# Shuijing725/CrowdNav_Prediction_AttnGraph

Hardware: AMD Instinct MI355X
Metric: env-steps/sec (sim+policy fwd) at 20 humans (higher is better)
Workload: dtype f32 (big GEMMs as bf16x3 split-precision MFMA, fp32 accumulate); 1 GPU; BASELINE configs[1]: CrowdSimVarNum-v0, 20 humans, 4096 parallel envs per GPU, HH+HR attention on, policy forward + ORCA sim step + auto-reset per step; envs_per_gpu=4096, humans=20, parallelism=dp1 (envs sharded, no rollout collective), policy_init=orthogonal, torch.manual_seed(425), sampled_actions=True, side_stream_tail=inline, dephase_steps=240

## Files before the change

crowdnav_prediction_attngraph_amd/csrc/common.h:

```cpp
#pragma once
#include <hip/hip_runtime.h>

#include <cstdarg>
#include <cstdint>
#include <cstdio>

#include "crowdnav_hip.h"

void cn_set_error(const char *fmt, ...);

#define CN_HIP(expr)                                                                                         \
    do {                                                                                                     \
        hipError_t cn_e_ = (expr);                                                                           \
        if (cn_e_ != hipSuccess) {                                                                           \
            cn_set_error("%s failed: %s (%s:%d)", #expr, hipGetErrorString(cn_e_), __FILE__, __LINE__);      \
            return CN_ERR_HIP;                                                                               \
        }                                                                                                    \
    } while (0)

#define CN_CHECK_LAUNCH() CN_HIP(hipGetLastError())

#define CN_REQUIRE(cond, ...)               \
    do {                                    \
        if (!(cond)) {                      \
// ... 82 lines not shown
    v = fmaxf(v, wv_dpp<0x118, 0xf>(v, I));
    v = fmaxf(v, wv_dpp<0x142, 0xa>(v, I));
    v = fmaxf(v, wv_dpp<0x143, 0xc>(v, I));
    return wv_readlane(v, 63);
}
__device__ __forceinline__ float wv_sum(float v)
{
    v += wv_dpp<0x111, 0xf>(v, 0.0f);
    v += wv_dpp<0x112, 0xf>(v, 0.0f);
    v += wv_dpp<0x114, 0xf>(v, 0.0f);
    v += wv_dpp<0x118, 0xf>(v, 0.0f);
    v += wv_dpp<0x142, 0xa>(v, 0.0f);
    v += wv_dpp<0x143, 0xc>(v, 0.0f);
    return wv_readlane(v, 63);
}
__device__ __forceinline__ double wv_min(double v)
{
#pragma unroll
    for (int o = 32; o > 0; o >>= 1) v = fmin(v, __shfl_xor(v, o, 64));
    return v;
}
__device__ __forceinline__ double wv_sum(double v)
{
#pragma unroll
    for (int o = 32; o > 0; o >>= 1) v += __shfl_xor(v, o, 64);
    return v;
}
```

crowdnav_prediction_attngraph_amd/csrc/det_math.h:

```cpp
#pragma once
#include "common.h"

#include <cmath>

namespace {

__device__ __forceinline__ double poly_sin(double x)
{
    const double S1 = -1.66666666666666324348e-01, S2 = 8.33333333332248946124e-03, S3 = -1.98412698298579493134e-04,
                 S4 = 2.75573137070700676789e-06, S5 = -2.50507602534068634195e-08, S6 = 1.58969099521155010221e-10;
    const double z = x * x, w = z * z;
    const double r = S2 + z * (S3 + z * S4) + z * w * (S5 + z * S6);
    const double v = z * x;
    return x + v * (S1 + z * r);
}
__device__ __forceinline__ double poly_cos(double x)
{
    const double C1 = 4.16666666666666019037e-02, C2 = -1.38888888888741095749e-03, C3 = 2.48015872894767294178e-05,
                 C4 = -2.75573143513906633035e-07, C5 = 2.08757232129817482790e-09, C6 = -1.13596475577881948265e-11;
    const double z = x * x;
    double w = z * z;
    const double r = z * (C1 + z * (C2 + z * C3)) + (w * w) * (C4 + z * (C5 + z * C6));
    const double hz = 0.5 * z;
    w = 1.0 - hz;
// ... 54 lines not shown
    }
    const double s = f / (2.0 + f);
    const double z = s * s;
    const double w = z * z;
    const double t1 = w * (Lg2 + w * (Lg4 + w * Lg6));
    const double t2 = z * (Lg1 + w * (Lg3 + w * (Lg5 + w * Lg7)));
    const double R = t2 + t1;
    const int i = (hx - 0x6147a) | (0x6b851 - hx);
    if (i > 0) {
        const double hfsq = 0.5 * f * f;
        return k == 0 ? f - (hfsq - s * (hfsq + R)) : dk * ln2_hi - ((hfsq - (s * (hfsq + R) + dk * ln2_lo)) - f);
    }
    return k == 0 ? f - s * (f - R) : dk * ln2_hi - ((s * (f - R) - dk * ln2_lo) - f);
}

__device__ __forceinline__ bool in_fov(const cn_env_config &c, double fov, double px1, double py1, double vx1, double vy1, double theta1,
                                       double px2, double py2)
{
    double fx, fy;
    if (c.kinematics == CN_KIN_UNICYCLE) det_sincos(theta1, fy, fx);
    else if (vx1 == 0.0 && vy1 == 0.0) { fx = __double_as_longlong(vx1) < 0 ? -1.0 : 1.0; fy = 0.0; }
    else { const double nv = sqrt(vx1 * vx1 + vy1 * vy1); fx = vx1 / nv; fy = vy1 / nv; }
    const double dx = px2 - px1, dy = py2 - py1;
    const double n12 = sqrt(dx * dx + dy * dy);
    double d = fx * (dx / n12) + fy * (dy / n12);
    d = d < -1.0 ? -1.0 : (d > 1.0 ? 1.0 : d);
    const double half = M_PI * fov / 2.0;
    double thr = -1.0;
    if (half < M_PI) { double sn; det_sincos(half, sn, thr); }
    return d >= thr;
}
// ... 3 lines not shown
```

crowdnav_prediction_attngraph_amd/csrc/env_dev.h:

```cpp
#pragma once
#include "common.h"

namespace {

constexpr int MT_N = 624;
constexpr float RVO_EPS = 0.00001f;

struct Lp3Hdr { int32_t agent, nn, line_fail; float rx, ry, radius; };

struct EnvDev {
    cn_env_config cfg;
    int E, H, D, P;
    int I, R;
    int64_t seed_base;
    double *hum;
    double *rob;
    double *lhs;
    double *ftraj;
    int32_t *step_counter;
    uint64_t *case_counter;
    double *ep_ret;
    int32_t *ep_cnt;
    double *shared_nd;
    uint8_t *sim_valid;
// ... 26 lines not shown
    int32_t *obs_max;
    uint8_t *sim_n;
    uint8_t *rob_sim_n;
    int32_t *pred_id;
    int32_t *max_pid;
    uint8_t *last_obs;
    int32_t *lp3_cnt;
    struct Lp3Hdr *lp3_hdr;
    float4 *lp3_lines;
    double *desired_v;
    double *wheel;
    unsigned long long *stamp;
};
static EnvDev stamped(const EnvDev &d, int kernel_id) { EnvDev c = d; c.stamp = cn_stamp_slot(kernel_id); return c; }

__device__ __forceinline__ int crowd_size(const EnvDev &s, int e) { return s.nh ? s.nh[e] : s.H; }

constexpr int CN_MAX_PLACEMENT_ATTEMPTS = 1 << 16;

enum { F_PX = 0, F_PY, F_VX, F_VY, F_GX, F_GY, F_RAD, F_VPREF };
enum { R_PX = 0, R_PY, R_VX, R_VY, R_GX, R_GY, R_THETA, R_POT };

}
```

crowdnav_prediction_attngraph_amd/csrc/env_sim.hip:

```cpp
#include "common.h"
#include "env_dev.h"
#include "det_math.h"
#include "orca.h"
#include "mt19937.h"
#include "episode.h"

#include <cmath>
#include <cstdio>
#include <cstdlib>
#include <cstring>
#include <new>

namespace {

__global__ __launch_bounds__(64) void env_reset_kernel(EnvDev s, cn_obs ob, int with_obs)
{
    const int lane = threadIdx.x;
    const int e = blockIdx.x;
    Rng R{MT_N, false};
    Robot rb{};
    Lane h{};
    h.rad = s.cfg.human_radius;
    double shared_nd = s.cfg.orca_neighbor_dist;
    int n = s.H;
    if (e == 0 && lane == 0) *s.lp3_cnt = 0;
    const bool nx_ready = s.nx_ready[e] != 0;
// ... 62 lines not shown
    Rng R{MT_N, false};
    Robot rb;
    Lane h;
    load_env(s, e, lane, rb, h);
    double shared_nd = s.shared_nd[e];
    const bool was_reset = s.pend[e] != 0;
    const int n = crowd_size(s, e);
    write_obs(s, e, lane, n, was_reset, rb, h, ob, was_reset ? 0 : s.step_counter[e]);
    if (!was_reset) post_obs_updates(s, R, e, lane, n, s.step_counter[e], rb, h, shared_nd);
    if (lane == 0) s.pend[e] = 0;
    store_env(s, e, lane, rb, h);
    if (lane == 0) s.shared_nd[e] = shared_nd;
    rng_store(R, s, e, lane);
}

template <bool SPLIT, int W = 1, bool DEFER = false>
__global__ __launch_bounds__(64 * W, W > 1 ? 2 : 4) void env_step_kernel(EnvDev s, const float *actions, cn_obs ob, float *reward_out,
                                                      uint8_t *done_out, uint8_t *info_out, double *ep_ret_out, int32_t *ep_len_out, float *not_done_out)
{
    const CnStampScope stamp_scope(s.stamp);
    const int lane = threadIdx.x & 63;
    const int e = blockIdx.x;
    if constexpr (W > 1) {
        if (threadIdx.x >= 64) { coop_helper_loop<W>(lane, __builtin_amdgcn_readfirstlane((int)(threadIdx.x >> 6))); return; }
    }
    const cn_env_config &c = s.cfg;
    const int H = s.H;
    const int lj = lane < H ? lane : 0;
    int n = crowd_size(s, e);
    Rng R{MT_N, false};
    Robot rb;
    Lane h;
    load_env(s, e, lane, rb, h);
    double shared_nd = s.shared_nd[e];
    int step_counter = s.step_counter[e];
    float ax = actions[2 * e], ay = actions[2 * e + 1];
    const float hax = s.hact[(size_t)e * 2 * H + lj], hay = s.hact[(size_t)e * 2 * H + H + lj];
    double ep_ret_in = s.ep_ret[e];
    int ep_cnt_in = s.ep_cnt[e];
    int nx_ready_in = s.nx_ready[e];
    uint64_t case_counter = s.case_counter[e];
// ... 107 lines not shown
            const bool hidden = c.human_fov < 2.0 ? !in_fov(c, c.human_fov, h.px, h.py, h.vx, h.vy, 0.0, ox, oy) : (ox == h.px && oy == h.py);
            if (hidden) { ox = 7.0; oy = 7.0; if (j < n) orad = c.human_radius; }
            const double dx = h.px - ox, dy = h.py - oy;
            const double d = sqrt(dx * dx + dy * dy);
            const double f = c.sf_A * det_exp((h.rad + orad - d) / c.sf_B);
            if (j != lane) { ivx += f * (dx / d); ivy += f * (dy / d); }
        }
        const double nvx = h.vx + (curr_dvx + ivx) * c.time_step, nvy = h.vy + (curr_dvy + ivy) * c.time_step;
        const double act_norm = sqrt(nvx * nvx + nvy * nvy);
        if (act_norm > h.vpref) { sfx = nvx / act_norm * h.vpref; sfy = nvy / act_norm * h.vpref; }
        else { sfx = nvx; sfy = nvy; }
    }
    const double cdx = h.px - rb.px, cdy = h.py - rb.py;
    const double closest = isH ? sqrt(cdx * cdx + cdy * cdy) - h.rad - c.robot_radius : INFINITY;
    const bool collision = wv_any(closest < 0.0);
    const double dmin = wv_min(closest);
    const double goal_dist = norm2(rb.px - rb.gx, rb.py - rb.gy);
    const bool reaching_goal = goal_dist < (c.kinematics == CN_KIN_UNICYCLE ? 0.6 : c.robot_radius);
    const double global_time = (double)step_counter * c.time_step;
    double reward;
    int done, info;
    const bool test_phase = c.phase == CN_PHASE_TEST;
    bool danger_cond = dmin < c.discomfort_dist;
    double min_danger = 0.0, rf_truth = 0.0;
    if (test_phase) {
        const double *tre = s.tr + (size_t)e * (s.R + 1) * 4 * H;
        const bool seen = isH && held(seen_before) != 0;
        double best = INFINITY;
        for (int k = 1; k <= s.P; ++k) {
            if (isH) {
                const double fx = (seen ? tre[(k * s.I * 4 + 0) * H + lane] : 15.0) - rb.px, fy = (seen ? tre[(k * s.I * 4 + 1) * H + lane] : 15.0) - rb.py;
// ... 249 lines not shown
}

static int truth_rollout_and_obs(cn_env_batch *env, const cn_obs *obs, hipStream_t st)
{
    if (int rc = truth_rollout(env, st)) return rc;
    hipLaunchKernelGGL(env_obs_kernel, dim3(env->d.E), dim3(64), 0, st, env->d, *obs);
    CN_CHECK_LAUNCH();
    return CN_OK;
}

static bool lane_path_of(const cn_env_batch *env)
{
    const int slots = env->d.H + (env->d.cfg.robot_visible ? 1 : 0);
    return env->d.cfg.humans_policy == CN_HUMANS_ORCA && slots <= 32 && env->d.cfg.human_fov >= 2.0;
}

static bool dense_crowd(cn_env_batch *env)
{
    const cn_env_config &cf = env->d.cfg;
    const double zone = 2.0 * (2.0 * (cf.randomize_attributes ? 0.5 : cf.human_radius) + cf.discomfort_dist) * env->d.H;
    static const int coop_env = getenv("CN_ENV_COOP") ? atoi(getenv("CN_ENV_COOP")) : -1;
    static const int coop_after = getenv("CN_COOP_AFTER") ? atoi(getenv("CN_COOP_AFTER")) : COOP_AFTER;
    env->d.coop_after = coop_after;
    return coop_env >= 0 ? coop_env != 0 : zone > 0.9 * 2.0 * M_PI * cf.circle_radius;
}

static int launch_post(cn_env_batch *env, hipStream_t on)
{
    hipLaunchKernelGGL(env_post_kernel<4>, dim3(env->d.E), dim3(256), 0, on, stamped(env->d, CN_K_OTHER));
    CN_CHECK_LAUNCH();
// ... 302 lines not shown
    if (!env->orca_ready && !env->tail_pending) { if (int rc = prefetch_orca(env, st, nullptr)) return rc; }
    if (int rc = sync_side(env, st)) return rc;
    if (env->d.cfg.predict_truth) {
        hipLaunchKernelGGL(env_step_kernel<true>, dim3(env->d.E), dim3(64), 0, st, stamped(env->d, CN_K_ENV_STEP), actions, *obs, reward, done, info, ep_return, ep_len, not_done);
        CN_CHECK_LAUNCH();
        if (int rc = truth_rollout_and_obs(env, obs, st)) return rc;
    } else {
        const bool coop = dense_crowd(env);
        const bool defer = coop && !lane_path_of(env) && env->d.cfg.humans_policy == CN_HUMANS_ORCA;
        if (defer) {
            CN_HIP(hipMemsetAsync(env->d.post_cnt, 0, 4, st));
            hipLaunchKernelGGL((env_step_kernel<false, 1, true>), dim3(env->d.E), dim3(64), 0, st, stamped(env->d, CN_K_ENV_STEP), actions, *obs, reward, done, info, ep_return, ep_len, not_done);
            env->post_deferred = true;
        }
        else if (coop) hipLaunchKernelGGL((env_step_kernel<false, 4>), dim3(env->d.E), dim3(256), 0, st, stamped(env->d, CN_K_ENV_STEP), actions, *obs, reward, done, info, ep_return, ep_len, not_done);
        else hipLaunchKernelGGL(env_step_kernel<false>, dim3(env->d.E), dim3(64), 0, st, stamped(env->d, CN_K_ENV_STEP), actions, *obs, reward, done, info, ep_return, ep_len, not_done);
        CN_CHECK_LAUNCH();
    }
    return prefetch_orca(env, st, obs);
}

extern "C" int cn_env_join(cn_env_batch *env, void *stream)
{
    CN_REQUIRE(env, "cn_env_join: null handle");
    return sync_side(env, (hipStream_t)stream);
}

extern "C" int cn_env_get_state(cn_env_batch *env, double *humans, double *robot, void *stream)
{
    CN_REQUIRE(env, "cn_env_get_state: null handle");
// ... 138 lines not shown
```

crowdnav_prediction_attngraph_amd/csrc/episode.h:

```cpp
#pragma once
#include "env_dev.h"
#include "det_math.h"
#include "mt19937.h"

namespace {

struct Lane {
    double px, py, vx, vy, gx, gy, rad, vpref;
    double l0, l1, l2, l3, l4;
    uint8_t simv;
};
struct Robot { double px, py, vx, vy, gx, gy, theta, pot; };

__device__ __forceinline__ double norm2(double x, double y) { return sqrt(x * x + y * y); }
__device__ __forceinline__ bool closer_than(double x, double y, double d)
{
    const double q = x * x + y * y, dd = d * d;
    if (q < dd * (1.0 - 0x1p-48)) return true;
    if (q > dd * (1.0 + 0x1p-48)) return false;
    return sqrt(q) < d;
}

__device__ __forceinline__ double wv_readlane_d(double v, int lane_uniform)
{
    const long long b = __double_as_longlong(v);
    const unsigned lo = (unsigned)__builtin_amdgcn_readlane((int)(unsigned)(b & 0xffffffffll), lane_uniform);
    const unsigned hi = (unsigned)__builtin_amdgcn_readlane((int)(unsigned)((unsigned long long)b >> 32), lane_uniform);
    return __longlong_as_double((long long)(((unsigned long long)hi << 32) | lo));
}

constexpr int coop_c(int W) { return W <= 4 ? 4 : (W <= 8 ? 2 : 1); }
template <int W>
struct CoopLds {
    static constexpr int NE = W - 1;
    static constexpr int C = coop_c(W);
    static constexpr int NG = NE * C;
    static constexpr int NB1 = (384 * NG + 623) / MT_N;
    static constexpr int BW = MT_N * (NB1 + 1) + 227;
    int cmd;
    int verdict;
    int kind, n_pairs, max_att;
    int pos0, attempt0;
    float circle_radius, vp;
// ... 71 lines not shown
        const float2 lo = Q.plo[k];
#pragma unroll
        for (int cc = 0; cc < C; ++cc) {
            const f2 ax = xx[cc] - f2{pq.x, pq.y}, ay = yy[cc] - f2{pq.z, pq.w};
            const f2 d = (ax * ax + ay * ay) - f2{lo.x, lo.y};
            m[cc] = fminf(m[cc], fminf(d.x, d.y));
        }
    }
#pragma unroll
    for (int cc = 0; cc < C; ++cc) {
        const uint64_t take = __ballot(!(m[cc] < 0.0f) || att0 + 64 * (p * C + cc) + lane >= max_att);
        if (lane == 0) Q.take[round & 1][p * C + cc] = take;
    }
}

template <int W = 1>
__device__ __forceinline__ void place_by_rejection(const EnvDev &s, Rng &R, int lane, int kind, double radius, double vp, double md_r, int n_list, int skip,
                                                   const Robot &rb, const Lane &h, double &out_x, double &out_y)
{
    const cn_env_config &c = s.cfg;
    const int max_att = c.max_placement_attempts > 0 ? c.max_placement_attempts : CN_MAX_PLACEMENT_ATTEMPTS;
    auto make = [&](double u0, double u1, double u2, double &x, double &y) {
        const double angle = u0 * M_PI * 2.0;
        const double nx = kind == 0 ? (0.0 + (1.0 - 0.0) * u1) * 2.0 : (u1 - 0.5) * vp;
        const double ny = kind == 0 ? (0.0 + (1.0 - 0.0) * u2) * 2.0 : (u2 - 0.5) * vp;
        double sn, cs;
        det_sincos(angle, sn, cs);
        x = c.circle_radius * cs + nx;
        y = c.circle_radius * sn + ny;
    };
    const double md_l = radius + h.rad + c.discomfort_dist, dd_l = md_l * md_l;
    const double lo_l = dd_l * (1.0 - 0x1p-48), hi_l = dd_l * (1.0 + 0x1p-48);
    const double ddr = md_r * md_r, lo_r = ddr * (1.0 - 0x1p-48), hi_r = ddr * (1.0 + 0x1p-48);
    auto collides_exact = [&](double x, double y) {
        bool coll = norm2(x - rb.px, y - rb.py) < md_r || norm2(x - rb.gx, y - rb.gy) < md_r;
// ... 290 lines not shown
#endif
            __syncthreads();
            unsigned long long any = 0ull;
            for (int p = 0; p < NG; ++p) any |= Q.take[round & 1][p];
            if (any) {
                __syncthreads();
                if (Q.verdict) break;
            }
            bprev = (g0 + 384 * NG - 1) / MT_N;
            g0 += 384 * NG;
            attempt += 64 * NG;
        }
    }
}

template <int W = 1>
__device__ __forceinline__ void gen_human(const EnvDev &s, Rng &R, int lane, int slot, int n_existing, const Robot &rb, Lane &h, double &shared_nd)
{
    const cn_env_config &c = s.cfg;
    double radius = c.human_radius, vpref = c.human_v_pref;
    if (c.randomize_attributes) {
        shared_nd = rng_uniform(R, lane, 5.0, 10.0);
        vpref = rng_uniform(R, lane, 0.5, 1.5);
        radius = rng_uniform(R, lane, 0.3, 0.5);
    }
    double px, py;
    const double md_r = c.kinematics == CN_KIN_UNICYCLE ? c.circle_radius / 2.0 : radius + c.robot_radius + c.discomfort_dist;
    place_by_rejection<W>(s, R, lane, 0, radius, 0.0, md_r, n_existing, -1, rb, h, px, py);
    if (lane == slot) {
        h.px = px; h.py = py; h.gx = -px; h.gy = -py; h.vx = 0.0; h.vy = 0.0; h.rad = radius; h.vpref = vpref;
        h.simv = 0;
    }
}

template <int W = 1>
__device__ __forceinline__ void change_goals(const EnvDev &s, Rng &R, int lane, int n, const Robot &rb, Lane &h, int only = -1)
{
    const cn_env_config &c = s.cfg;
    const int H = n;
    for (int i = only >= 0 ? only : 0; i < (only >= 0 ? only + 1 : H); ++i) {
        double vp_i = __shfl(h.vpref, i, 64);
        const double rad_i = __shfl(h.rad, i, 64);
        if (only < 0 && vp_i == 0.0) continue;
        if (vp_i == 0.0) vp_i = 1.0;
        if (rng_double(R, lane) <= (only >= 0 ? c.end_goal_change_chance : c.goal_change_chance)) {
            double gx, gy;
            place_by_rejection<W>(s, R, lane, 1, rad_i, vp_i, rad_i + c.robot_radius + c.discomfort_dist, H, i, rb, h, gx, gy);
            if (lane == i) { h.gx = gx; h.gy = gy; }
        }
    }
}

__device__ __forceinline__ bool robot_sees(const cn_env_config &c, const Robot &rb, bool present, double hpx, double hpy, double hrad)
{
    const double dx = rb.px - hpx, dy = rb.py - hpy;
    bool vis = present && !(dx == 0.0 && dy == 0.0) && (norm2(dx, dy) - c.robot_radius - hrad <= c.sensor_range);
    if (c.robot_fov < 2.0) vis = vis && in_fov(c, c.robot_fov, rb.px, rb.py, rb.vx, rb.vy, rb.theta, hpx, hpy);
    return vis;
}

__device__ __forceinline__ void write_obs(const EnvDev &s, int e, int lane, int n, bool reset, const Robot &rb, Lane &h, const cn_obs &ob, int step_counter)
{
    const cn_env_config &c = s.cfg;
    const int H = s.H, D = s.D, P = s.P;
    const bool isH = lane < n, isRow = lane < H;
    const bool vis = robot_sees(c, rb, isH, h.px, h.py, h.rad);
    const uint64_t vmask = __ballot(vis);
    const int num_visible = __popcll(vmask);
    if (s.vis && isRow) s.vis[(size_t)e * H + lane] = vis ? 1 : 0;
    if (s.nh && c.env_kind != CN_ENV_PRED && lane == 0) {
        s.obs_cnt[e] = num_visible;
        s.obs_max[e] = vmask ? 63 - __clzll((long long)vmask) : -1;
    }
    const double prev_vx = h.l2, prev_vy = h.l3;
    if (vis) { h.l0 = h.px; h.l1 = h.py; h.l2 = h.vx; h.l3 = h.vy; h.l4 = h.rad; }
    else if (isH && reset) { h.l0 = 15.0; h.l1 = 15.0; h.l2 = 0.0; h.l3 = 0.0; h.l4 = 0.3; }
    else if (isH) { h.l0 = h.l0 + h.l2 * c.time_step; h.l1 = h.l1 + h.l3 * c.time_step; }
    if (lane == 0) {
// ... 18 lines not shown
            se[1] = (float)pid;
            se[2] = vis ? (float)h.l0 : INFINITY;
            se[3] = vis ? (float)h.l1 : INFINITY;
            if (ob.visible_masks) ob.visible_masks[(size_t)e * H + lane] = vis ? 1 : 0;
        }
        if (lane == 0 && omask) s.max_pid[e] = base + __popcll(omask);
        return;
    }
    const double ex = h.l0 - rb.px, ey = h.l1 - rb.py;
    const bool do_sort = c.sort_humans && c.env_kind != CN_ENV_PRED_GST;
    int row = lane;
    if (do_sort) {
        const double key = vis ? sqrt(ex * ex + ey * ey) : INFINITY;
        int rank = 0;
        for (int m = 0; m < H; ++m) {
            const double km = __shfl(key, m, 64);
            rank += (km < key || (km == key && m < lane)) ? 1 : 0;
        }
        row = rank;
    }
    if (isRow) {
        float *se = ob.spatial_edges + ((size_t)e * H + row) * D;
        if (c.env_kind == CN_ENV_VARNUM) {
            se[0] = vis ? (float)ex : 15.0f;
            se[1] = vis ? (float)ey : 15.0f;
        } else {
            double *ft = s.ftraj ? s.ftraj + (size_t)e * P * 2 * H : nullptr;
            const double *tre = c.predict_truth ? s.tr + (size_t)e * (s.R + 1) * 4 * H : nullptr;
            for (int k = 0; k <= P; ++k) {
                double fx = 15.0, fy = 15.0;
                if (vis && tre && k >= 1) {
// ... 10 lines not shown
                    se[2 * k + 1] = vis ? (float)(fy - rb.py) : 15.0f;
                } else {
                    se[2 * k] = vis ? (float)ex : 15.0f;
                    se[2 * k + 1] = vis ? (float)ey : 15.0f;
                }
            }
        }
        if (ob.visible_masks) {
            uint8_t *vm = ob.visible_masks + (size_t)e * H;
            if (do_sort) vm[lane] = lane < num_visible ? 1 : 0;
            else vm[lane] = vis ? 1 : 0;
        }
    }
}

__device__ __forceinline__ void gen_episode_head(const EnvDev &s, Rng &R, int e, int lane, uint64_t case_counter, Robot &rb, int &n)
{
    const cn_env_config &c = s.cfg;
    const uint64_t offset = c.phase == CN_PHASE_TRAIN ? 2000ull : (c.phase == CN_PHASE_VAL ? 0ull : 1000ull);
    const uint64_t seed = offset + case_counter + (uint64_t)(s.seed_base + e);
    rng_seed(R, (uint32_t)seed, lane);
    double px, py, gx, gy;
    if (c.kinematics == CN_KIN_UNICYCLE) {
        const double angle = rng_uniform(R, lane, 0.0, M_PI * 2.0);
        double sn, cs;
        det_sincos(angle, sn, cs);
        px = c.arena_size * cs; py = c.arena_size * sn;
        for (;;) {
            gx = rng_uniform(R, lane, -c.arena_size, c.arena_size);
            gy = rng_uniform(R, lane, -c.arena_size, c.arena_size);
            if (norm2(px - gx, py - gy) >= 4.0) break;
        }
        rb.theta = rng_uniform(R, lane, 0.0, 2.0 * M_PI);
        n = rng_randint(R, lane, 1, c.human_num + c.human_num_range + 1);
    } else {
        for (;;) {
            px = rng_uniform(R, lane, -c.arena_size, c.arena_size);
            py = rng_uniform(R, lane, -c.arena_size, c.arena_size);
            gx = rng_uniform(R, lane, -c.arena_size, c.arena_size);
            gy = rng_uniform(R, lane, -c.arena_size, c.arena_size);
            if (norm2(px - gx, py - gy) >= 8.0) break;
        }
        rb.theta = M_PI / 2.0;
        n = rng_randint(R, lane, c.human_num - c.human_num_range, c.human_num + c.human_num_range + 1);
    }
    rb.px = px; rb.py = py; rb.gx = gx; rb.gy = gy; rb.vx = 0.0; rb.vy = 0.0;
}
__device__ __forceinline__ void gen_episode(const EnvDev &s, Rng &R, int e, int lane, uint64_t case_counter, Robot &rb, Lane &h, double &shared_nd, int &n)
{
    gen_episode_head(s, R, e, lane, case_counter, rb, n);
    for (int i = 0; i < n; ++i) gen_human(s, R, lane, i, i, rb, h, shared_nd);
    rb.pot = -fabs(norm2(rb.gx - rb.px, rb.gy - rb.py));
}

__device__ __forceinline__ void finish_reset(const EnvDev &s, int e, int lane, int n, uint64_t case_counter, Robot &rb, Lane &h, const cn_obs &ob, bool with_obs = true)
{
    const cn_env_config &c = s.cfg;
    h.l0 = h.l1 = h.l2 = h.l3 = h.l4 = 0.0;
    const uint64_t case_size = c.phase == CN_PHASE_TRAIN ? (4294967295ull - 2000ull) : (c.phase == CN_PHASE_VAL ? c.val_size : c.test_size);
    if (lane == 0) {
        s.case_counter[e] = (case_counter + (uint64_t)c.nenv) % case_size;
        s.step_counter[e] = 0; s.ep_ret[e] = 0.0; s.ep_cnt[e] = 0;
        if (s.nh) { s.obs_cnt[e] = 0; s.obs_max[e] = -1; }
        if (s.max_pid) s.max_pid[e] = n;
        if (s.wheel) { s.wheel[(size_t)e * 4 + 2] = 0.0; s.wheel[(size_t)e * 4 + 3] = 0.0; }
    }
    if (s.pred_id && lane < s.H) { s.pred_id[(size_t)e * s.H + lane] = lane; s.last_obs[(size_t)e * s.H + lane] = 0; }
    if (with_obs) write_obs(s, e, lane, n, true, rb, h, ob, 0);
}

__device__ __forceinline__ void do_reset(const EnvDev &s, Rng &R, int e, int lane, bool nx_ready, uint64_t case_counter, Robot &rb, Lane &h,
                                         double &shared_nd, int &n, const cn_obs &ob, bool with_obs = true)
{
    if (nx_ready) {
        rng_sync();
        mt_dma(R.mt, s.nx_mt + (size_t)e * MT_N, lane);
        const int pos = s.nx_mt_pos[e];
        n = s.nx_nh ? s.nx_nh[e] : s.H;
        const int H = s.H;
        const int lj = lane < H ? lane : 0;
        const double *hum = s.nx_hum + (size_t)e * 8 * H;
        h.px = hum[F_PX * H + lj]; h.py = hum[F_PY * H + lj]; h.vx = 0.0; h.vy = 0.0;
        h.gx = hum[F_GX * H + lj]; h.gy = hum[F_GY * H + lj]; h.rad = hum[F_RAD * H + lj]; h.vpref = hum[F_VPREF * H + lj];
        h.simv = 0;
        const double *r = s.nx_rob + (size_t)e * 8;
        rb.px = r[R_PX]; rb.py = r[R_PY]; rb.vx = 0.0; rb.vy = 0.0; rb.gx = r[R_GX]; rb.gy = r[R_GY]; rb.theta = r[R_THETA]; rb.pot = r[R_POT];
        shared_nd = s.nx_shared_nd[e];
        mt_dma_wait();
        R.pos = pos;
        R.loaded = true;
        rng_sync();
        if (lane == 0) s.nx_ready[e] = 0;
    } else {
        gen_episode(s, R, e, lane, case_counter, rb, h, shared_nd, n);
    }
    finish_reset(s, e, lane, n, case_counter, rb, h, ob, with_obs);
}

__device__ __forceinline__ void load_env(const EnvDev &s, int e, int lane, Robot &rb, Lane &h)
{
    const int H = s.H;
    const int lj = lane < H ? lane : 0;
    const double *hum = s.hum + (size_t)e * 8 * H;
    h.px = hum[F_PX * H + lj]; h.py = hum[F_PY * H + lj]; h.vx = hum[F_VX * H + lj]; h.vy = hum[F_VY * H + lj];
    h.gx = hum[F_GX * H + lj]; h.gy = hum[F_GY * H + lj]; h.rad = hum[F_RAD * H + lj]; h.vpref = hum[F_VPREF * H + lj];
    const double *l = s.lhs + (size_t)e * 5 * H;
    h.l0 = l[lj]; h.l1 = l[H + lj]; h.l2 = l[2 * H + lj]; h.l3 = l[3 * H + lj]; h.l4 = l[4 * H + lj];
    h.simv = s.sim_valid[(size_t)e * H + lj];
    const double *r = s.rob + (size_t)e * 8;
    rb.px = r[R_PX]; rb.py = r[R_PY]; rb.vx = r[R_VX]; rb.vy = r[R_VY]; rb.gx = r[R_GX]; rb.gy = r[R_GY]; rb.theta = r[R_THETA]; rb.pot = r[R_POT];
}
__device__ __forceinline__ void store_env(const EnvDev &s, int e, int lane, const Robot &rb, const Lane &h)
{
    const int H = s.H;
    if (lane < H) {
        double *hum = s.hum + (size_t)e * 8 * H;
        hum[F_PX * H + lane] = h.px; hum[F_PY * H + lane] = h.py; hum[F_VX * H + lane] = h.vx; hum[F_VY * H + lane] = h.vy;
        hum[F_GX * H + lane] = h.gx; hum[F_GY * H + lane] = h.gy; hum[F_RAD * H + lane] = h.rad; hum[F_VPREF * H + lane] = h.vpref;
        double *l = s.lhs + (size_t)e * 5 * H;
        l[lane] = h.l0; l[H + lane] = h.l1; l[2 * H + lane] = h.l2; l[3 * H + lane] = h.l3; l[4 * H + lane] = h.l4;
        s.sim_valid[(size_t)e * H + lane] = h.simv;
    }
    if (lane == 0) {
        double *r = s.rob + (size_t)e * 8;
        r[R_PX] = rb.px; r[R_PY] = rb.py; r[R_VX] = rb.vx; r[R_VY] = rb.vy; r[R_GX] = rb.gx; r[R_GY] = rb.gy; r[R_THETA] = rb.theta; r[R_POT] = rb.pot;
    }
}

template <int W = 1>
__device__ __forceinline__ void pregen_env(const EnvDev &s, int e, int lane, long long budget, Rng &R)
{
    if (s.nx_ready[e]) return;
    const long long t0 = wall_clock64();
    const int H = s.H;
    int prog = s.nx_prog[e];
    if (prog > 0 && s.nx_case[e] != s.case_counter[e]) prog = 0;
    Robot rb{};
    Lane h{};
    h.rad = s.cfg.human_radius;
    double shared_nd = s.shared_nd[e];
    int n = H;
    if (prog == 0) {
        const uint64_t case_counter = s.case_counter[e];
        gen_episode_head(s, R, e, lane, case_counter, rb, n);
        if (lane == 0) s.nx_case[e] = case_counter;
// ... 26 lines not shown
    }
    if (lane == 0) {
        double *r = s.nx_rob + (size_t)e * 8;
        r[R_PX] = rb.px; r[R_PY] = rb.py; r[R_GX] = rb.gx; r[R_GY] = rb.gy; r[R_THETA] = rb.theta; r[R_POT] = rb.pot;
        s.nx_shared_nd[e] = shared_nd;
        s.nx_mt_pos[e] = R.pos;
        if (s.nx_nh) s.nx_nh[e] = n;
        s.nx_prog[e] = complete ? 0 : prog;
    }
    rng_sync();
    for (int k = lane; k < MT_N; k += 64) s.nx_mt[(size_t)e * MT_N + k] = R.mt[k];
    __threadfence();
    if (lane == 0 && complete) s.nx_ready[e] = 1;
}

template <int W = 1>
__device__ __forceinline__ void post_obs_updates(const EnvDev &s, Rng &R, int e, int lane, int n, int step_counter, const Robot &rb, Lane &h, double &shared_nd)
{
    const cn_env_config &c = s.cfg;
    const int H = n;
    const bool isH = lane < H;
    const int period = (int)(5.0 / c.time_step + 0.5);
    if (c.random_goal_changing && (step_counter % period) == 0) {
        rng_load(R, s, e, lane);
        change_goals<W>(s, R, lane, n, rb, h);
    }
    if (c.end_goal_changing) {
        uint64_t reached = __ballot(isH && norm2(h.gx - h.px, h.gy - h.py) < h.rad);
        if (reached) rng_load(R, s, e, lane);
        while (reached) {
            const int i = __ffsll((unsigned long long)reached) - 1;
            reached &= reached - 1;
            if (c.kinematics == CN_KIN_UNICYCLE && c.env_kind == CN_ENV_VARNUM) change_goals<W>(s, R, lane, n, rb, h, i);
            else gen_human<W>(s, R, lane, i, H, rb, h, shared_nd);
// ... 6 lines not shown
```

crowdnav_prediction_attngraph_amd/csrc/mt19937.h:

```cpp
#pragma once
#include "env_dev.h"
#include "det_math.h"

namespace {

__shared__ uint32_t g_mt_lds[MT_N];
struct Rng {
    int pos;
    bool loaded;
    uint32_t *mt = g_mt_lds;
    bool pre_ok = false;
    int pre_pos = 0;
};
__device__ __forceinline__ void rng_sync()
{
    __builtin_amdgcn_fence(__ATOMIC_SEQ_CST, "wavefront");
    __builtin_amdgcn_wave_barrier();
    __builtin_amdgcn_fence(__ATOMIC_SEQ_CST, "wavefront");
}

__device__ __forceinline__ void mt_dma(uint32_t *dst, const uint32_t *src, int lane)
{
    typedef __attribute__((address_space(3))) uint32_t lds_u32;
    typedef __attribute__((address_space(1))) const uint32_t glb_u32;
    asm volatile("s_waitcnt lgkmcnt(0)" ::: "memory");
#pragma unroll
    for (int t = 0; t < (MT_N + 63) / 64; ++t)
        if (lane + 64 * t < MT_N) __builtin_amdgcn_global_load_lds((glb_u32 *)(src + lane + 64 * t), (lds_u32 *)(dst + 64 * t), 4, 0, 0);
}
__device__ __forceinline__ void mt_dma_wait() { asm volatile("s_waitcnt vmcnt(0)" ::: "memory"); }

__device__ __forceinline__ void rng_prefetch(Rng &R, const EnvDev &s, int e, int lane)
{
    if (R.loaded || R.pre_ok) return;
    mt_dma(R.mt, s.mt + (size_t)e * MT_N, lane);
    R.pre_pos = s.mt_pos[e];
    R.pre_ok = true;
}
__device__ __forceinline__ void rng_load(Rng &R, const EnvDev &s, int e, int lane)
{
    if (R.loaded) return;
    if (R.pre_ok) {
        mt_dma_wait();
        R.pos = held(R.pre_pos);
    } else {
        for (int k = lane; k < MT_N; k += 64) R.mt[k] = s.mt[(size_t)e * MT_N + k];
        R.pos = s.mt_pos[e];
    }
    R.loaded = true;
    rng_sync();
}
__device__ __forceinline__ void rng_store(Rng &R, const EnvDev &s, int e, int lane)
{
    if (!R.loaded) return;
    rng_sync();
    for (int k = lane; k < MT_N; k += 64) s.mt[(size_t)e * MT_N + k] = R.mt[k];
    if (lane == 0) s.mt_pos[e] = R.pos;
}
__device__ __forceinline__ void rng_seed(Rng &R, uint32_t seed, int lane)
{
    rng_sync();
    uint32_t sd = (uint32_t)__builtin_amdgcn_readfirstlane((int)seed);
    for (int base = 0; base < MT_N; base += 64) {
        uint32_t mine = 0;
        for (int t = 0; t < 64; ++t) {
            const int pos = base + t;
            if (pos < MT_N) {
// ... 99 lines not shown
```

Baseline: 15.69 million env-steps/s.

## Specialize env step kernel for the training profile with compile-time config constants

Adds a ProfileTrain view whose config fields such as env kind, kinematics, policy and FOV are constexpr and whose optional pointers are constexpr null. The host launches this specialized env_step kernel when the runtime config matches, and device helpers are templated on the view type. The intent is to let the compiler drop dead branches and loads for unused features. It also swaps the double wave-min and sort-rank shuffles for DPP and readlane forms in the pinned path. The cost is extra code size, an additional kernel instantiation, and the need to keep the profile check in sync with the config.

```diff
diff --git a/crowdnav_prediction_attngraph_amd/csrc/common.h b/crowdnav_prediction_attngraph_amd/csrc/common.h
--- a/crowdnav_prediction_attngraph_amd/csrc/common.h
+++ b/crowdnav_prediction_attngraph_amd/csrc/common.h
@@ -120,6 +120,32 @@
     v += wv_dpp<0x143, 0xc>(v, 0.0f);
     return wv_readlane(v, 63);
 }
+__device__ __forceinline__ double wv_readlane_d(double v, int lane_uniform)
+{
+    const long long b = __double_as_longlong(v);
+    const unsigned lo = (unsigned)__builtin_amdgcn_readlane((int)(unsigned)(b & 0xffffffffll), lane_uniform);
+    const unsigned hi = (unsigned)__builtin_amdgcn_readlane((int)(unsigned)((unsigned long long)b >> 32), lane_uniform);
+    return __longlong_as_double((long long)(((unsigned long long)hi << 32) | lo));
+}
+template <int CTRL, int ROW_MASK>
+__device__ __forceinline__ double wv_dpp(double v, double identity)
+{
+    const unsigned long long b = (unsigned long long)__double_as_longlong(v), id = (unsigned long long)__double_as_longlong(identity);
+    const unsigned lo = (unsigned)__builtin_amdgcn_update_dpp((int)(unsigned)id, (int)(unsigned)b, CTRL, ROW_MASK, 0xf, false);
+    const unsigned hi = (unsigned)__builtin_amdgcn_update_dpp((int)(unsigned)(id >> 32), (int)(unsigned)(b >> 32), CTRL, ROW_MASK, 0xf, false);
+    return __longlong_as_double((long long)(((unsigned long long)hi << 32) | lo));
+}
+__device__ __forceinline__ double wv_min_dpp(double v)
+{
+    const double I = __builtin_inf();
+    v = fmin(v, wv_dpp<0x111, 0xf>(v, I));
+    v = fmin(v, wv_dpp<0x112, 0xf>(v, I));
+    v = fmin(v, wv_dpp<0x114, 0xf>(v, I));
+    v = fmin(v, wv_dpp<0x118, 0xf>(v, I));
+    v = fmin(v, wv_dpp<0x142, 0xa>(v, I));
+    v = fmin(v, wv_dpp<0x143, 0xc>(v, I));
+    return wv_readlane_d(v, 63);
+}
 __device__ __forceinline__ double wv_min(double v)
 {
 #pragma unroll
diff --git a/crowdnav_prediction_attngraph_amd/csrc/det_math.h b/crowdnav_prediction_attngraph_amd/csrc/det_math.h
--- a/crowdnav_prediction_attngraph_amd/csrc/det_math.h
+++ b/crowdnav_prediction_attngraph_amd/csrc/det_math.h
@@ -92,7 +92,8 @@
     return k == 0 ? f - s * (f - R) : dk * ln2_hi - ((s * (f - R) - dk * ln2_lo) - f);
 }
 
-__device__ __forceinline__ bool in_fov(const cn_env_config &c, double fov, double px1, double py1, double vx1, double vy1, double theta1,
+template <class C>
+__device__ __forceinline__ bool in_fov(const C &c, double fov, double px1, double py1, double vx1, double vy1, double theta1,
                                        double px2, double py2)
 {
     double fx, fy;
diff --git a/crowdnav_prediction_attngraph_amd/csrc/env_dev.h b/crowdnav_prediction_attngraph_amd/csrc/env_dev.h
--- a/crowdnav_prediction_attngraph_amd/csrc/env_dev.h
+++ b/crowdnav_prediction_attngraph_amd/csrc/env_dev.h
@@ -64,7 +64,8 @@
 };
 static EnvDev stamped(const EnvDev &d, int kernel_id) { EnvDev c = d; c.stamp = cn_stamp_slot(kernel_id); return c; }
 
-__device__ __forceinline__ int crowd_size(const EnvDev &s, int e) { return s.nh ? s.nh[e] : s.H; }
+template <class S>
+__device__ __forceinline__ int crowd_size(const S &s, int e) { return s.nh ? s.nh[e] : s.H; }
 
 constexpr int CN_MAX_PLACEMENT_ATTEMPTS = 1 << 16;
 
diff --git a/crowdnav_prediction_attngraph_amd/csrc/env_profile.h b/crowdnav_prediction_attngraph_amd/csrc/env_profile.h
--- /dev/null
+++ b/crowdnav_prediction_attngraph_amd/csrc/env_profile.h
@@ -0,0 +1,105 @@
+#pragma once
+#include "env_dev.h"
+
+namespace {
+
+struct ProfileGeneric {};
+struct ProfileTrain {};
+
+struct CfgTrain {
+    static constexpr int32_t env_kind = CN_ENV_VARNUM;
+    static constexpr int32_t randomize_attributes = 0;
+    static constexpr int32_t phase = CN_PHASE_TRAIN;
+    static constexpr int32_t robot_policy = CN_ROBOT_NETWORK;
+    static constexpr int32_t robot_visible = 0;
+    static constexpr int32_t predict_truth = 0;
+    static constexpr int32_t human_num_range = 0;
+    static constexpr int32_t kinematics = CN_KIN_HOLONOMIC;
+    static constexpr int32_t humans_policy = CN_HUMANS_ORCA;
+    static constexpr double robot_fov = 2.0, human_fov = 2.0;
+    const int32_t &human_num, &predict_steps, &random_goal_changing, &end_goal_changing, &sort_humans, &nenv;
+    const uint32_t &val_size, &test_size;
+    const int32_t &auto_reset, &max_placement_attempts, &pred_interval;
+    const double &time_step, &time_limit, &success_reward, &collision_penalty, &discomfort_dist, &discomfort_penalty_factor;
+    const double &circle_radius, &arena_size, &human_radius, &human_v_pref, &robot_radius, &robot_v_pref, &sensor_range;
+    const double &goal_change_chance, &end_goal_change_chance;
+    const double &orca_neighbor_dist, &orca_safety_space, &orca_time_horizon, &orca_time_horizon_obst;
+    const double &sf_A, &sf_B, &sf_KI;
+    __host__ __device__ explicit CfgTrain(const cn_env_config &c)
+        : human_num(c.human_num), predict_steps(c.predict_steps), random_goal_changing(c.random_goal_changing),
+          end_goal_changing(c.end_goal_changing), sort_humans(c.sort_humans), nenv(c.nenv), val_size(c.val_size), test_size(c.test_size),
+          auto_reset(c.auto_reset), max_placement_attempts(c.max_placement_attempts), pred_interval(c.pred_interval),
+          time_step(c.time_step), time_limit(c.time_limit), success_reward(c.success_reward), collision_penalty(c.collision_penalty),
+          discomfort_dist(c.discomfort_dist), discomfort_penalty_factor(c.discomfort_penalty_factor), circle_radius(c.circle_radius),
+          arena_size(c.arena_size), human_radius(c.human_radius), human_v_pref(c.human_v_pref), robot_radius(c.robot_radius),
+          robot_v_pref(c.robot_v_pref), sensor_range(c.sensor_range), goal_change_chance(c.goal_change_chance),
+          end_goal_change_chance(c.end_goal_change_chance), orca_neighbor_dist(c.orca_neighbor_dist), orca_safety_space(c.orca_safety_space),
+          orca_time_horizon(c.orca_time_horizon), orca_time_horizon_obst(c.orca_time_horizon_obst), sf_A(c.sf_A), sf_B(c.sf_B), sf_KI(c.sf_KI)
+    {
+    }
+};
+
+struct EnvTrain {
+    const CfgTrain cfg;
+    static constexpr int D = 2;
+    const int &E, &H, &P, &I, &R;
+    const int64_t &seed_base;
+    static constexpr double *ftraj = nullptr, *tr = nullptr, *desired_v = nullptr, *wheel = nullptr;
+    static constexpr float *sim_seen = nullptr, *rob_nd = nullptr, *rob_seen = nullptr;
+    static constexpr uint8_t *vis = nullptr, *sim_n = nullptr, *rob_sim_n = nullptr, *rob_sim_valid = nullptr, *last_obs = nullptr;
+    static constexpr int32_t *nh = nullptr, *nx_nh = nullptr, *obs_cnt = nullptr, *obs_max = nullptr, *pred_id = nullptr, *max_pid = nullptr;
+    double *const &hum, *const &rob, *const &lhs;
+    int32_t *const &step_counter;
+    uint64_t *const &case_counter;
+    double *const &ep_ret;
+    int32_t *const &ep_cnt;
+    double *const &shared_nd;
+    uint8_t *const &sim_valid;
+    float *const &sim_nd, *const &sim_self_radius, *const &sim_self_maxspeed;
+    uint32_t *const &mt;
+    int32_t *const &mt_pos;
+    float *const &hact;
+    double *const &nx_hum, *const &nx_rob, *const &nx_shared_nd;
+    uint32_t *const &nx_mt;
+    int32_t *const &nx_mt_pos, *const &post_cnt, *const &post_list, *const &plan_arrive;
+    const int &coop_after;
+    uint8_t *const &nx_ready;
+    int32_t *const &nx_prog;
+    uint64_t *const &nx_case;
+    double *const &min_dist;
+    uint8_t *const &pend;
+    int32_t *const &lp3_cnt;
+    Lp3Hdr *const &lp3_hdr;
+    float4 *const &lp3_lines;
+    unsigned long long *const &stamp;
+    __host__ __device__ explicit EnvTrain(const EnvDev &d)
+        : cfg(d.cfg), E(d.E), H(d.H), P(d.P), I(d.I), R(d.R), seed_base(d.seed_base), hum(d.hum), rob(d.rob), lhs(d.lhs),
+          step_counter(d.step_counter), case_counter(d.case_counter), ep_ret(d.ep_ret), ep_cnt(d.ep_cnt), shared_nd(d.shared_nd),
+          sim_valid(d.sim_valid), sim_nd(d.sim_nd), sim_self_radius(d.sim_self_radius), sim_self_maxspeed(d.sim_self_maxspeed), mt(d.mt),
+          mt_pos(d.mt_pos), hact(d.hact), nx_hum(d.nx_hum), nx_rob(d.nx_rob), nx_shared_nd(d.nx_shared_nd), nx_mt(d.nx_mt),
+          nx_mt_pos(d.nx_mt_pos), post_cnt(d.post_cnt), post_list(d.post_list), plan_arrive(d.plan_arrive), coop_after(d.coop_after),
+          nx_ready(d.nx_ready), nx_prog(d.nx_prog), nx_case(d.nx_case), min_dist(d.min_dist), pend(d.pend), lp3_cnt(d.lp3_cnt),
+          lp3_hdr(d.lp3_hdr), lp3_lines(d.lp3_lines), stamp(d.stamp)
+    {
+    }
+};
+
+static bool train_profile_of(const EnvDev &d)
+{
+    const cn_env_config &c = d.cfg;
+    return c.env_kind == CfgTrain::env_kind && c.randomize_attributes == CfgTrain::randomize_attributes && c.phase == CfgTrain::phase &&
+           c.robot_policy == CfgTrain::robot_policy && c.robot_visible == CfgTrain::robot_visible && c.predict_truth == CfgTrain::predict_truth &&
+           c.human_num_range == CfgTrain::human_num_range && c.kinematics == CfgTrain::kinematics && c.humans_policy == CfgTrain::humans_policy &&
+           c.robot_fov >= 2.0 && c.human_fov >= 2.0 && d.D == EnvTrain::D &&
+           !d.ftraj && !d.tr && !d.desired_v && !d.wheel && !d.sim_seen && !d.rob_nd && !d.rob_seen && !d.vis && !d.sim_n && !d.rob_sim_n &&
+           !d.rob_sim_valid && !d.last_obs && !d.nh && !d.nx_nh && !d.obs_cnt && !d.obs_max && !d.pred_id && !d.max_pid;
+}
+
+template <class PF> struct EnvViewOf;
+template <> struct EnvViewOf<ProfileGeneric> { typedef const EnvDev &type; };
+template <> struct EnvViewOf<ProfileTrain> { typedef const EnvTrain type; };
+
+template <class S> constexpr bool view_pinned = false;
+template <> constexpr bool view_pinned<EnvTrain> = true;
+
+}
diff --git a/crowdnav_prediction_attngraph_amd/csrc/env_sim.hip b/crowdnav_prediction_attngraph_amd/csrc/env_sim.hip
--- a/crowdnav_prediction_attngraph_amd/csrc/env_sim.hip
+++ b/crowdnav_prediction_attngraph_amd/csrc/env_sim.hip
@@ -1,5 +1,6 @@
 #include "common.h"
 #include "env_dev.h"
+#include "env_profile.h"
 #include "det_math.h"
 #include "orca.h"
 #include "mt19937.h"
@@ -10,6 +11,7 @@
 #include <cstdlib>
 #include <cstring>
 #include <new>
+#include <type_traits>
 
 namespace {
 
@@ -102,17 +104,19 @@
     rng_store(R, s, e, lane);
 }
 
-template <bool SPLIT, int W = 1, bool DEFER = false>
-__global__ __launch_bounds__(64 * W, W > 1 ? 2 : 4) void env_step_kernel(EnvDev s, const float *actions, cn_obs ob, float *reward_out,
+template <bool SPLIT, int W = 1, bool DEFER = false, class PF = ProfileGeneric>
+__global__ __launch_bounds__(64 * W, W > 1 ? 2 : 4) void env_step_kernel(EnvDev s_arg, const float *actions, cn_obs ob, float *reward_out,
                                                       uint8_t *done_out, uint8_t *info_out, double *ep_ret_out, int32_t *ep_len_out, float *not_done_out)
 {
+    typename EnvViewOf<PF>::type s(s_arg);
+    typedef typename std::decay<decltype(s)>::type View;
     const CnStampScope stamp_scope(s.stamp);
     const int lane = threadIdx.x & 63;
     const int e = blockIdx.x;
     if constexpr (W > 1) {
         if (threadIdx.x >= 64) { coop_helper_loop<W>(lane, __builtin_amdgcn_readfirstlane((int)(threadIdx.x >> 6))); return; }
     }
-    const cn_env_config &c = s.cfg;
+    const auto &c = s.cfg;
     const int H = s.H;
     const int lj = lane < H ? lane : 0;
     int n = crowd_size(s, e);
@@ -250,7 +254,9 @@
     const double cdx = h.px - rb.px, cdy = h.py - rb.py;
     const double closest = isH ? sqrt(cdx * cdx + cdy * cdy) - h.rad - c.robot_radius : INFINITY;
     const bool collision = wv_any(closest < 0.0);
-    const double dmin = wv_min(closest);
+    double dmin;
+    if constexpr (view_pinned<View>) dmin = wv_min_dpp(closest);
+    else dmin = wv_min(closest);
     const double goal_dist = norm2(rb.px - rb.gx, rb.py - rb.gy);
     const bool reaching_goal = goal_dist < (c.kinematics == CN_KIN_UNICYCLE ? 0.6 : c.robot_radius);
     const double global_time = (double)step_counter * c.time_step;
@@ -530,6 +536,8 @@
     const int slots = env->d.H + (env->d.cfg.robot_visible ? 1 : 0);
     return env->d.cfg.humans_policy == CN_HUMANS_ORCA && slots <= 32 && env->d.cfg.human_fov >= 2.0;
 }
+
+static bool train_profile(const cn_env_batch *env) { return train_profile_of(env->d); }
 
 static bool dense_crowd(cn_env_batch *env)
 {
@@ -862,6 +870,7 @@
             env->post_deferred = true;
         }
         else if (coop) hipLaunchKernelGGL((env_step_kernel<false, 4>), dim3(env->d.E), dim3(256), 0, st, stamped(env->d, CN_K_ENV_STEP), actions, *obs, reward, done, info, ep_return, ep_len, not_done);
+        else if (train_profile(env)) hipLaunchKernelGGL((env_step_kernel<false, 1, false, ProfileTrain>), dim3(env->d.E), dim3(64), 0, st, stamped(env->d, CN_K_ENV_STEP), actions, *obs, reward, done, info, ep_return, ep_len, not_done);
         else hipLaunchKernelGGL(env_step_kernel<false>, dim3(env->d.E), dim3(64), 0, st, stamped(env->d, CN_K_ENV_STEP), actions, *obs, reward, done, info, ep_return, ep_len, not_done);
         CN_CHECK_LAUNCH();
     }
diff --git a/crowdnav_prediction_attngraph_amd/csrc/episode.h b/crowdnav_prediction_attngraph_amd/csrc/episode.h
--- a/crowdnav_prediction_attngraph_amd/csrc/episode.h
+++ b/crowdnav_prediction_attngraph_amd/csrc/episode.h
@@ -1,5 +1,6 @@
 #pragma once
 #include "env_dev.h"
+#include "env_profile.h"
 #include "det_math.h"
 #include "mt19937.h"
 
@@ -19,14 +20,6 @@
     if (q < dd * (1.0 - 0x1p-48)) return true;
     if (q > dd * (1.0 + 0x1p-48)) return false;
     return sqrt(q) < d;
-}
-
-__device__ __forceinline__ double wv_readlane_d(double v, int lane_uniform)
-{
-    const long long b = __double_as_longlong(v);
-    const unsigned lo = (unsigned)__builtin_amdgcn_readlane((int)(unsigned)(b & 0xffffffffll), lane_uniform);
-    const unsigned hi = (unsigned)__builtin_amdgcn_readlane((int)(unsigned)((unsigned long long)b >> 32), lane_uniform);
-    return __longlong_as_double((long long)(((unsigned long long)hi << 32) | lo));
 }
 
 constexpr int coop_c(int W) { return W <= 4 ? 4 : (W <= 8 ? 2 : 1); }
@@ -128,11 +121,11 @@
     }
 }
 
-template <int W = 1>
-__device__ __forceinline__ void place_by_rejection(const EnvDev &s, Rng &R, int lane, int kind, double radius, double vp, double md_r, int n_list, int skip,
+template <int W = 1, class S>
+__device__ __forceinline__ void place_by_rejection(const S &s, Rng &R, int lane, int kind, double radius, double vp, double md_r, int n_list, int skip,
                                                    const Robot &rb, const Lane &h, double &out_x, double &out_y)
 {
-    const cn_env_config &c = s.cfg;
+    const auto &c = s.cfg;
     const int max_att = c.max_placement_attempts > 0 ? c.max_placement_attempts : CN_MAX_PLACEMENT_ATTEMPTS;
     auto make = [&](double u0, double u1, double u2, double &x, double &y) {
         const double angle = u0 * M_PI * 2.0;
@@ -453,10 +446,10 @@
     }
 }
 
-template <int W = 1>
-__device__ __forceinline__ void gen_human(const EnvDev &s, Rng &R, int lane, int slot, int n_existing, const Robot &rb, Lane &h, double &shared_nd)
-{
-    const cn_env_config &c = s.cfg;
+template <int W = 1, class S>
+__device__ __forceinline__ void gen_human(const S &s, Rng &R, int lane, int slot, int n_existing, const Robot &rb, Lane &h, double &shared_nd)
+{
+    const auto &c = s.cfg;
     double radius = c.human_radius, vpref = c.human_v_pref;
     if (c.randomize_attributes) {
         shared_nd = rng_uniform(R, lane, 5.0, 10.0);
@@ -472,10 +465,10 @@
     }
 }
 
-template <int W = 1>
-__device__ __forceinline__ void change_goals(const EnvDev &s, Rng &R, int lane, int n, const Robot &rb, Lane &h, int only = -1)
-{
-    const cn_env_config &c = s.cfg;
+template <int W = 1, class S>
+__device__ __forceinline__ void change_goals(const S &s, Rng &R, int lane, int n, const Robot &rb, Lane &h, int only = -1)
+{
+    const auto &c = s.cfg;
     const int H = n;
     for (int i = only >= 0 ? only : 0; i < (only >= 0 ? only + 1 : H); ++i) {
         double vp_i = __shfl(h.vpref, i, 64);
@@ -490,7 +483,8 @@
     }
 }
 
-__device__ __forceinline__ bool robot_sees(const cn_env_config &c, const Robot &rb, bool present, double hpx, double hpy, double hrad)
+template <class C>
+__device__ __forceinline__ bool robot_sees(const C &c, const Robot &rb, bool present, double hpx, double hpy, double hrad)
 {
     const double dx = rb.px - hpx, dy = rb.py - hpy;
     bool vis = present && !(dx == 0.0 && dy == 0.0) && (norm2(dx, dy) - c.robot_radius - hrad <= c.sensor_range);
@@ -498,9 +492,10 @@
     return vis;
 }
 
-__device__ __forceinline__ void write_obs(const EnvDev &s, int e, int lane, int n, bool reset, const Robot &rb, Lane &h, const cn_obs &ob, int step_counter)
-{
-    const cn_env_config &c = s.cfg;
+template <class S>
+__device__ __forceinline__ void write_obs(const S &s, int e, int lane, int n, bool reset, const Robot &rb, Lane &h, const cn_obs &ob, int step_counter)
+{
+    const auto &c = s.cfg;
     const int H = s.H, D = s.D, P = s.P;
     const bool isH = lane < n, isRow = lane < H;
     const bool vis = robot_sees(c, rb, isH, h.px, h.py, h.rad);
@@ -549,7 +544,9 @@
         const double key = vis ? sqrt(ex * ex + ey * ey) : INFINITY;
         int rank = 0;
         for (int m = 0; m < H; ++m) {
-            const double km = __shfl(key, m, 64);
+            double km;
+            if constexpr (view_pinned<S>) km = wv_readlane_d(key, m);
+            else km = __shfl(key, m, 64);
             rank += (km < key || (km == key && m < lane)) ? 1 : 0;
         }
         row = rank;
@@ -590,9 +587,10 @@
     }
 }
 
-__device__ __forceinline__ void gen_episode_head(const EnvDev &s, Rng &R, int e, int lane, uint64_t case_counter, Robot &rb, int &n)
-{
-    const cn_env_config &c = s.cfg;
+template <class S>
+__device__ __forceinline__ void gen_episode_head(const S &s, Rng &R, int e, int lane, uint64_t case_counter, Robot &rb, int &n)
+{
+    const auto &c = s.cfg;
     const uint64_t offset = c.phase == CN_PHASE_TRAIN ? 2000ull : (c.phase == CN_PHASE_VAL ? 0ull : 1000ull);
     const uint64_t seed = offset + case_counter + (uint64_t)(s.seed_base + e);
     rng_seed(R, (uint32_t)seed, lane);
@@ -622,16 +620,18 @@
     }
     rb.px = px; rb.py = py; rb.gx = gx; rb.gy = gy; rb.vx = 0.0; rb.vy = 0.0;
 }
-__device__ __forceinline__ void gen_episode(const EnvDev &s, Rng &R, int e, int lane, uint64_t case_counter, Robot &rb, Lane &h, double &shared_nd, int &n)
+template <class S>
+__device__ __forceinline__ void gen_episode(const S &s, Rng &R, int e, int lane, uint64_t case_counter, Robot &rb, Lane &h, double &shared_nd, int &n)
 {
     gen_episode_head(s, R, e, lane, case_counter, rb, n);
     for (int i = 0; i < n; ++i) gen_human(s, R, lane, i, i, rb, h, shared_nd);
     rb.pot = -fabs(norm2(rb.gx - rb.px, rb.gy - rb.py));
 }
 
-__device__ __forceinline__ void finish_reset(const EnvDev &s, int e, int lane, int n, uint64_t case_counter, Robot &rb, Lane &h, const cn_obs &ob, bool with_obs = true)
-{
-    const cn_env_config &c = s.cfg;
+template <class S>
+__device__ __forceinline__ void finish_reset(const S &s, int e, int lane, int n, uint64_t case_counter, Robot &rb, Lane &h, const cn_obs &ob, bool with_obs = true)
+{
+    const auto &c = s.cfg;
     h.l0 = h.l1 = h.l2 = h.l3 = h.l4 = 0.0;
     const uint64_t case_size = c.phase == CN_PHASE_TRAIN ? (4294967295ull - 2000ull) : (c.phase == CN_PHASE_VAL ? c.val_size : c.test_size);
     if (lane == 0) {
@@ -645,7 +645,8 @@
     if (with_obs) write_obs(s, e, lane, n, true, rb, h, ob, 0);
 }
 
-__device__ __forceinline__ void do_reset(const EnvDev &s, Rng &R, int e, int lane, bool nx_ready, uint64_t case_counter, Robot &rb, Lane &h,
+template <class S>
+__device__ __forceinline__ void do_reset(const S &s, Rng &R, int e, int lane, bool nx_ready, uint64_t case_counter, Robot &rb, Lane &h,
                                          double &shared_nd, int &n, const cn_obs &ob, bool with_obs = true)
 {
     if (nx_ready) {
@@ -673,7 +674,8 @@
     finish_reset(s, e, lane, n, case_counter, rb, h, ob, with_obs);
 }
 
-__device__ __forceinline__ void load_env(const EnvDev &s, int e, int lane, Robot &rb, Lane &h)
+template <class S>
+__device__ __forceinline__ void load_env(const S &s, int e, int lane, Robot &rb, Lane &h)
 {
     const int H = s.H;
     const int lj = lane < H ? lane : 0;
@@ -686,7 +688,8 @@
     const double *r = s.rob + (size_t)e * 8;
     rb.px = r[R_PX]; rb.py = r[R_PY]; rb.vx = r[R_VX]; rb.vy = r[R_VY]; rb.gx = r[R_GX]; rb.gy = r[R_GY]; rb.theta = r[R_THETA]; rb.pot = r[R_POT];
 }
-__device__ __forceinline__ void store_env(const EnvDev &s, int e, int lane, const Robot &rb, const Lane &h)
+template <class S>
+__device__ __forceinline__ void store_env(const S &s, int e, int lane, const Robot &rb, const Lane &h)
 {
     const int H = s.H;
     if (lane < H) {
@@ -703,8 +706,8 @@
     }
 }
 
-template <int W = 1>
-__device__ __forceinline__ void pregen_env(const EnvDev &s, int e, int lane, long long budget, Rng &R)
+template <int W = 1, class S>
+__device__ __forceinline__ void pregen_env(const S &s, int e, int lane, long long budget, Rng &R)
 {
     if (s.nx_ready[e]) return;
     const long long t0 = wall_clock64();
@@ -761,10 +764,10 @@
     if (lane == 0 && complete) s.nx_ready[e] = 1;
 }
 
-template <int W = 1>
-__device__ __forceinline__ void post_obs_updates(const EnvDev &s, Rng &R, int e, int lane, int n, int step_counter, const Robot &rb, Lane &h, double &shared_nd)
-{
-    const cn_env_config &c = s.cfg;
+template <int W = 1, class S>
+__device__ __forceinline__ void post_obs_updates(const S &s, Rng &R, int e, int lane, int n, int step_counter, const Robot &rb, Lane &h, double &shared_nd)
+{
+    const auto &c = s.cfg;
     const int H = n;
     const bool isH = lane < H;
     const int period = (int)(5.0 / c.time_step + 0.5);
diff --git a/crowdnav_prediction_attngraph_amd/csrc/mt19937.h b/crowdnav_prediction_attngraph_amd/csrc/mt19937.h
--- a/crowdnav_prediction_attngraph_amd/csrc/mt19937.h
+++ b/crowdnav_prediction_attngraph_amd/csrc/mt19937.h
@@ -30,14 +30,16 @@
 }
 __device__ __forceinline__ void mt_dma_wait() { asm volatile("s_waitcnt vmcnt(0)" ::: "memory"); }
 
-__device__ __forceinline__ void rng_prefetch(Rng &R, const EnvDev &s, int e, int lane)
+template <class S>
+__device__ __forceinline__ void rng_prefetch(Rng &R, const S &s, int e, int lane)
 {
     if (R.loaded || R.pre_ok) return;
     mt_dma(R.mt, s.mt + (size_t)e * MT_N, lane);
     R.pre_pos = s.mt_pos[e];
     R.pre_ok = true;
 }
-__device__ __forceinline__ void rng_load(Rng &R, const EnvDev &s, int e, int lane)
+template <class S>
+__device__ __forceinline__ void rng_load(Rng &R, const S &s, int e, int lane)
 {
     if (R.loaded) return;
     if (R.pre_ok) {
@@ -50,7 +52,8 @@
     R.loaded = true;
     rng_sync();
 }
-__device__ __forceinline__ void rng_store(Rng &R, const EnvDev &s, int e, int lane)
+template <class S>
+__device__ __forceinline__ void rng_store(Rng &R, const S &s, int e, int lane)
 {
     if (!R.loaded) return;
     rng_sync();
```

After: 15.93 million env-steps/s, median of 6. 1.5% higher.
